# bjack205/rsLQR

Hardware: AMD Instinct MI355X
Metric: LQR solves/sec (nx=12,nu=4,N=256,batch=1024 per GPU) (higher is better)
Workload: dtype f64; 1 GPU; nx=12 nu=4 N=256 batch=1024 per GPU, fp64, factor+solve per step; parallelism=batch-sharded x1, no data-path collective, ranks_seen=1, flags=0, schedule=reduced-fused2

## Files before the change

### rslqr_amd/build.py

```python
import concurrent.futures
import os
import re
import shutil
import subprocess
import sys

PKG = os.path.dirname(os.path.abspath(__file__))
ROOT = os.path.dirname(PKG)
CSRC = os.path.join(PKG, "csrc")
INCLUDE = os.path.join(ROOT, "include")
OBJDIR = os.path.join(PKG, "build")
LIB = os.path.join(PKG, "librslqr_amd.so")
ARCH = "gfx950"

C_SOURCES = ["containers.c", "synth.c", "json.c", "batch.c", "solver.c", "linalg.c", "stages.c"]
HIP_MAIN = "ndlqr_hip.hip"
HIP_INSTANCE = "small_instance.hip"
HIP_DEPS = ["kernels_common.hpp", "kernels_leaf.hpp", "kernels_generic.hpp", "kernels_grad.hpp", "kernels_box.hpp", "kernels_box_grad.hpp", "kernels_small.hpp", "kernels_bottom_reduced.hpp", "kernels_dpp.hpp", "kernels_rowbcast.hpp", "kernels_mfma.hpp", "kernels_reduced_mfma.hpp",
            "hip_context.hpp", "launch_small.hpp", "small_instances.def"]


def small_instances():
    text = open(os.path.join(CSRC, "small_instances.def")).read()
    return [(int(a), int(b)) for a, b in re.findall(r"^NDLQR_SMALL_INSTANCE\((\d+),\s*(\d+)\)", text, flags=re.M)]


def _hipcc():
    for cand in (os.environ.get("HIPCC"), shutil.which("hipcc"), "/opt/rocm/bin/hipcc"):
        if cand and os.path.exists(cand):
            return cand
    raise RuntimeError("hipcc not found (set HIPCC)")


def _newer(target, deps):
    if not os.path.exists(target):
        return True
    t = os.path.getmtime(target)
    return any(os.path.exists(d) and os.path.getmtime(d) > t for d in deps)


def _run(cmd):
    proc = subprocess.run(cmd, stdout=subprocess.PIPE, stderr=subprocess.STDOUT, text=True)
    if proc.returncode != 0:
        sys.stderr.write(" ".join(cmd) + "\n" + proc.stdout + "\n")
        raise RuntimeError("build step failed: " + cmd[0])
    if proc.stdout.strip():
        sys.stderr.write(proc.stdout)


def build(force=False, verbose=False):
    os.makedirs(OBJDIR, exist_ok=True)
    headers = [os.path.join(INCLUDE, h) for h in ("ndlqr.h", "ndlqr_hip.h")]
    me = os.path.abspath(__file__)
    hipcc = _hipcc()
    hip_flags = [hipcc, "--offload-arch=" + ARCH, "-std=c++17", "-O3", "-ffp-contract=off", "-fPIC", "-Wall",
                 "-Wno-pass-failed",
                 "-I" + INCLUDE, "-I" + CSRC] + os.environ.get("NDLQR_EXTRA_HIPFLAGS", "").split()
    hip_deps = [me] + headers + [os.path.join(CSRC, h) for h in HIP_DEPS]
    jobs, objs = [], []
    for src in C_SOURCES:
        s = os.path.join(CSRC, src)
        o = os.path.join(OBJDIR, src + ".o")
        if force or _newer(o, [s, me] + headers):
            jobs.append(("cc " + src, ["gcc", "-std=gnu11", "-O2", "-g0", "-fPIC", "-Wall", "-Wextra",
                                       "-I" + INCLUDE, "-c", s, "-o", o]))
        objs.append(o)
    s = os.path.join(CSRC, HIP_MAIN)
    o = os.path.join(OBJDIR, HIP_MAIN + ".o")
    if force or _newer(o, [s] + hip_deps):
        jobs.append(("hipcc " + HIP_MAIN, hip_flags + ["-c", s, "-o", o]))
    objs.append(o)
    s = os.path.join(CSRC, HIP_INSTANCE)
    for nx, nu in small_instances():
        o = os.path.join(OBJDIR, "small_%d_%d.o" % (nx, nu))
        if force or _newer(o, [s] + hip_deps):
            jobs.append(("hipcc small instance (%d,%d)" % (nx, nu),
                         hip_flags + ["-DNDLQR_INST_NX=%d" % nx, "-DNDLQR_INST_NU=%d" % nu, "-c", s, "-o", o]))
        objs.append(o)
    if jobs:
        workers = max(1, min(len(jobs), (os.cpu_count() or 2)))
        with concurrent.futures.ThreadPoolExecutor(max_workers=workers) as pool:
            futures = {pool.submit(_run, cmd): label for label, cmd in jobs}
            for fut in concurrent.futures.as_completed(futures):
                fut.result()
                if verbose:
                    print(futures[fut])
    if force or _newer(LIB, objs):
        if verbose:
            print("link", os.path.basename(LIB))
        _run([hipcc, "--offload-arch=" + ARCH, "-shared", "-fPIC", "-o", LIB] + objs + ["-lm", "-lpthread"])
    return LIB


if __name__ == "__main__":
    print(build(force="--force" in sys.argv, verbose=True))
```

### rslqr_amd/csrc/kernels_bottom_reduced.hpp

```cpp
#pragma once
#include "kernels_dpp.hpp"
#include "kernels_small.hpp"

namespace ndlqr {

typedef double acc4_t __attribute__((ext_vector_type(4)));

template <int NX>
struct McPitch {
  static constexpr int SP = 18, WP = 17;
};

template <int NX, class Hook>
__device__ __forceinline__ void factor_tail_mc(const int lane, const acc4_t& c, const double (&ra)[(NX + 3) / 4],
                                               const double (&rb)[(NX + 3) / 4], const double* Wm, acc4_t& X0,
                                               acc4_t& X1, Hook hook) {
  constexpr int KS = (NX + 3) / 4, WP = McPitch<NX>::WP;
  int lane_o = lane;
  asm volatile("" : "+v"(lane_o));
  const int li = lane_o & 15, lk = lane_o >> 4;
  double wt[KS], wa[KS], b0[KS];
#pragma unroll
  for (int q = 0; q < KS; ++q) {
    wt[q] = Wm[(4 * q + lk) * WP + li];
    wa[q] = Wm[li * WP + 4 * q + lk];
    b0[q] = li == NX ? c[q] : ra[q];
  }
  const acc4_t zero = {0.0, 0.0, 0.0, 0.0};
  acc4_t Y0 = zero, Y1 = zero;
#pragma unroll
  for (int q = 0; q < KS; ++q) {
    Y0 = __builtin_amdgcn_mfma_f64_16x16x4f64(wa[q], b0[q], Y0, 0, 0, 0);
    Y1 = __builtin_amdgcn_mfma_f64_16x16x4f64(wa[q], rb[q], Y1, 0, 0, 0);
  }
  X0 = zero; X1 = zero;
  double y0[KS], y1[KS];
#pragma unroll
  for (int q = 0; q < KS; ++q) {
    y0[q] = Y0[q]; y1[q] = Y1[q];
    X0 = __builtin_amdgcn_mfma_f64_16x16x4f64(wt[q], Y0[q], X0, 0, 0, 0);
    X1 = __builtin_amdgcn_mfma_f64_16x16x4f64(wt[q], Y1[q], X1, 0, 0, 0);
  }
  hook(y0, y1, Y0, Y1);
}

template <int NX>
struct McWyLayout {
  static constexpr int SP = McPitch<NX>::SP, WP = McPitch<NX>::WP, KS = (NX + 3) / 4, YP = 17, TILE = 4 * KS * YP;
  static constexpr int Y0 = 0, Y1 = TILE, W = 2 * TILE;
  static constexpr int SIZE = 2 * TILE + 16 * WP > 16 * SP ? 2 * TILE + 16 * WP : 16 * SP;
  static_assert(2 * NX + 1 <= 32, "the panel fits the lanes of two DPP rows");
};
template <int NX>
__device__ __forceinline__ bool chol_wy_mc(const int lane_in, const acc4_t& c, double* buf, double (&w)[NX],
                                           double* lstore) {
  using P = McWyLayout<NX>;
  constexpr int SP = P::SP, YP = P::YP, KS = P::KS;
  static_assert(P::YP == P::WP, "one store stride for both kinds of lanes");
  int lane = lane_in;
  asm volatile("" : "+v"(lane));
  const int li = lane & 15, lk = lane >> 4, h = lane & 31;
  const int ri = li < NX ? li : NX - 1;
#pragma unroll
  for (int g = 0; g < 4; ++g) buf[(lk + 4 * g) * SP + li] = c[g];
  wave_lds_sync();
  double acc[NX];
  if constexpr (NX % 2 == 0) {
#pragma unroll
    for (int j = 0; j < NX; j += 2) {
      const double2 t = *reinterpret_cast<const double2*>(&buf[ri * SP + j]);
      acc[j] = t.x; acc[j + 1] = t.y;
    }
  } else {
#pragma unroll
    for (int j = 0; j < NX; ++j) acc[j] = buf[ri * SP + j];
  }
  if (lk >= 2) {
#pragma unroll
    for (int k = 0; k < NX; ++k) w[k] = (k == li) ? 1.0 : 0.0;
  } else if (h == NX) {
#pragma unroll
    for (int k = 0; k < NX; ++k) w[k] = buf[k * SP + NX];
  }
  const bool bad = rb_chol_inv<NX, false>(li, acc, w);
  wave_lds_sync();
  {
    const int ycol = h <= NX ? P::Y0 + h : P::Y1 + (h <= 2 * NX ? h - NX - 1 : YP - 1);
    double* dst = buf + (lk < 2 ? ycol : P::W + li);
#pragma unroll
    for (int k = 0; k < NX; ++k) dst[k * YP] = w[k];
    if constexpr (4 * KS > NX) {
#pragma unroll
      for (int e0 = 0; e0 < (4 * KS - NX) * YP; e0 += 32) {
        const int e = e0 + h;
        if (e < (4 * KS - NX) * YP && lk < 2) {
          buf[P::Y0 + NX * YP + e] = 0.0;
          buf[P::Y1 + NX * YP + e] = 0.0;
        }
      }
    }
#pragma unroll
    for (int e0 = 0; e0 < (16 - NX) * P::WP; e0 += 32) {
      const int e = e0 + h;
      if (e < (16 - NX) * P::WP && lk >= 2) buf[P::W + NX * P::WP + e] = 0.0;
    }
  }
  if (lstore && lane < NX) store_row<NX>(lstore + li * NX, acc);
  wave_lds_sync();
  return bad;
}

template <int NX, class Hook>
__device__ __forceinline__ void tail_wy_mc(const int lane, const double* buf, acc4_t& X0, acc4_t& X1, Hook hook) {
  using P = McWyLayout<NX>;
  constexpr int KS = P::KS;
  int lane_o = lane;
  asm volatile("" : "+v"(lane_o));
  const int li = lane_o & 15, lk = lane_o >> 4;
  double wt[KS], y0[KS], y1[KS];
  acc4_t Z0 = {0.0, 0.0, 0.0, 0.0}, Z1 = {0.0, 0.0, 0.0, 0.0};
#pragma unroll
  for (int q = 0; q < KS; ++q) {
    wt[q] = buf[P::W + (4 * q + lk) * P::WP + li];
    y0[q] = buf[P::Y0 + (4 * q + lk) * P::YP + li];
    y1[q] = buf[P::Y1 + (4 * q + lk) * P::YP + li];
    Z0[q] = y0[q]; Z1[q] = y1[q];
  }
  const acc4_t zero = {0.0, 0.0, 0.0, 0.0};
  X0 = zero; X1 = zero;
#pragma unroll
  for (int q = 0; q < KS; ++q) {
    X0 = __builtin_amdgcn_mfma_f64_16x16x4f64(wt[q], y0[q], X0, 0, 0, 0);
    X1 = __builtin_amdgcn_mfma_f64_16x16x4f64(wt[q], y1[q], X1, 0, 0, 0);
  }
  hook(y0, y1, Z0, Z1);
}

template <int NX>
struct McPairLayout {
  static constexpr int SP = McPitch<NX>::SP, WP = McPitch<NX>::WP;
  static constexpr int SCR_A = 0, SCR_B = 16 * SP, W_A = 32 * SP, W_B = 0, SIZE = 32 * SP + 16 * WP;
  static_assert(16 * WP <= 16 * SP, "W_B fits over the S-bar tile of A");
};
template <int NX>
__device__ __forceinline__ bool chol_pair_mc(const int lane_in, const acc4_t& cA, const acc4_t& cB, double* buf,
                                             double* lstoreA, double* lstoreB) {
  using P = McPairLayout<NX>;
  constexpr int SP = P::SP, WP = P::WP;
  int lane = lane_in;
  asm volatile("" : "+v"(lane));
  const int li = lane & 15, lk = lane >> 4;
  const int ri = li < NX ? li : NX - 1;
#pragma unroll
  for (int g = 0; g < 4; ++g) {
    buf[P::SCR_A + (lk + 4 * g) * SP + li] = cA[g];
    buf[P::SCR_B + (lk + 4 * g) * SP + li] = cB[g];
  }
  wave_lds_sync();
  const double* mine = buf + (lk < 2 ? P::SCR_A : P::SCR_B) + ri * SP;
  double acc[NX], w[NX];
  if constexpr (NX % 2 == 0) {
#pragma unroll
    for (int j = 0; j < NX; j += 2) {
      const double2 t = *reinterpret_cast<const double2*>(&mine[j]);
      acc[j] = t.x; acc[j + 1] = t.y;
    }
  } else {
#pragma unroll
    for (int j = 0; j < NX; ++j) acc[j] = mine[j];
  }
  const bool bad = rb_chol_inv<NX>(li, acc, w);
  wave_lds_sync();
  {
    double* wdst = buf + (lk < 2 ? P::W_A : P::W_B) + li;
#pragma unroll
    for (int r = 0; r < NX; ++r) wdst[r * WP] = w[r];
#pragma unroll
    for (int e0 = 0; e0 < (16 - NX) * WP; e0 += 32) {
      const int e = e0 + (lane & 31);
      if (e < (16 - NX) * WP) buf[(lk < 2 ? P::W_A : P::W_B) + NX * WP + e] = 0.0;
    }
  }
  if (lstoreA && lane < NX) store_row<NX>(lstoreA + li * NX, acc);
  if (lstoreB && lane >= 32 && lane < 32 + NX) store_row<NX>(lstoreB + li * NX, acc);
  wave_lds_sync();
  return bad;
}
// ... 42 lines not shown
    const int x = lk >> 1;
    double* ydst = buf + (h <= NX ? P::tile(x, 0) + h : P::tile(x, 1) + (h <= 2 * NX ? h - NX - 1 : YP - 1));
#pragma unroll
    for (int k = 0; k < NX; ++k) ydst[k * YP] = w[k];
    if constexpr (4 * KS > NX) {
#pragma unroll
      for (int e0 = 0; e0 < (4 * KS - NX) * YP; e0 += 16) {
        const int e = e0 + li;
        if (e < (4 * KS - NX) * YP) buf[P::tile(x, lk & 1) + NX * YP + e] = 0.0;
      }
    }
  }
  if ((lk & 1) == 0 && li < NX) {
    double* lr = (lk == 0 ? lrecA : lrecB) + li * (li + 1) / 2;
#pragma unroll
    for (int c = 0; c < NX; ++c)
      if (c <= li) lr[c] = acc[c];
  }
  wave_lds_sync();
  return bad;
}

template <int NX, bool N00, bool N01, bool N10, bool N11>
__device__ __forceinline__ void gram_mc(const double (&R0)[(NX + 3) / 4], const double (&R1)[(NX + 3) / 4],
                                        const acc4_t& X0, const acc4_t& X1, acc4_t& g00, acc4_t& g01, acc4_t& g10,
                                        acc4_t& g11) {
  constexpr int KS = (NX + 3) / 4;
  const acc4_t zero = {0.0, 0.0, 0.0, 0.0};
  g00 = zero; g01 = zero; g10 = zero; g11 = zero;
#pragma unroll
  for (int q = 0; q < KS; ++q) {
    if constexpr (N00) g00 = __builtin_amdgcn_mfma_f64_16x16x4f64(R0[q], X0[q], g00, 0, 0, 0);
    if constexpr (N01) g01 = __builtin_amdgcn_mfma_f64_16x16x4f64(R0[q], X1[q], g01, 0, 0, 0);
    if constexpr (N10) g10 = __builtin_amdgcn_mfma_f64_16x16x4f64(R1[q], X0[q], g10, 0, 0, 0);
    if constexpr (N11) g11 = __builtin_amdgcn_mfma_f64_16x16x4f64(R1[q], X1[q], g11, 0, 0, 0);
  }
}

template <int NX> __device__ __forceinline__ constexpr bool rows_all(int g) { return 4 * g + 3 < NX; }
template <int NX> __device__ __forceinline__ constexpr bool rows_none(int g) { return 4 * g >= NX; }

template <int NX>
__device__ __forceinline__ void store_record_mc(double* __restrict__ myrec, const int lane, const bool ha,
                                                const bool hb, const acc4_t& X0, const acc4_t& X1) {
  constexpr int NN = NX * NX;
  const int li = lane & 15, lk = lane >> 4;
  if (li < NX) {
    if (ha) {
#pragma unroll
      for (int g = 0; g < 4; ++g) {
        const int r = lk + 4 * g;
        if (!rows_none<NX>(g) && (rows_all<NX>(g) || r < NX)) myrec[r * NX + li] = X0[g];
      }
    }
    if (hb) {
#pragma unroll
      for (int g = 0; g < 4; ++g) {
        const int r = lk + 4 * g;
        if (!rows_none<NX>(g) && (rows_all<NX>(g) || r < NX)) myrec[NN + r * NX + li] = X1[g];
      }
    }
  } else if (li == NX) {
#pragma unroll
    for (int g = 0; g < 4; ++g) {
      const int r = lk + 4 * g;
      if (!rows_none<NX>(g) && (rows_all<NX>(g) || r < NX)) myrec[2 * NN + r] = X0[g];
    }
  }
}

struct StorePlain { __device__ __forceinline__ void operator()(double* p, double v) const { *p = v; } };
struct StoreThrough {
  __device__ __forceinline__ void operator()(double* p, double v) const {
    __hip_atomic_store(p, v, __ATOMIC_RELAXED, __HIP_MEMORY_SCOPE_AGENT);
  }
};
struct AddAtomic { __device__ __forceinline__ void operator()(double* p, double v) const { atomicAdd(p, v); } };

template <int NX, class Put, class Set>
__device__ __forceinline__ void push_mc(const int lane, const bool hasA, const bool hasB, const bool leftchild,
                                        const RedSlot<NX>& sa, const RedSlot<NX>& sb, const acc4_t& g00,
                                        const acc4_t& g01, const acc4_t& g11, const acc4_t& pa, const acc4_t& pb01,
                                        const acc4_t& pb11, Put put, Set set) {
  const int li = lane & 15, lk = lane >> 4;
  if (hasA && li <= NX) {
#pragma unroll
    for (int g = 0; g < 4; ++g) {
      const int r = lk + 4 * g;
      if (!rows_none<NX>(g) && (rows_all<NX>(g) || r < NX) && (li <= r || li == NX))
        put(li < NX ? sa.DR() + r * (r + 1) / 2 + li : sa.gR() + r, g00[g] + pa[g]);
    }
  }
  if (hasB && li < NX) {
#pragma unroll
    for (int g = 0; g < 4; ++g) {
      const int r = lk + 4 * g;
      if (!rows_none<NX>(g) && (rows_all<NX>(g) || r < NX) && li <= r) put(sb.DL() + r * (r + 1) / 2 + li, g11[g] + pb11[g]);
    }
    if (lk == NX % 4) put(sb.gL() + li, g01[NX / 4] + pb01[NX / 4]);
    if (hasA) {
#pragma unroll
      for (int g = 0; g < 4; ++g) {
        const int r = lk + 4 * g;
        if (!rows_none<NX>(g) && (rows_all<NX>(g) || r < NX))
          set(leftchild ? sb.CA() + li * NX + r : sa.CB() + r * NX + li, g01[g]);
      }
    }
  }
}

template <int NX, int NU, int WP, bool NEXT = true, class Init>
__device__ __forceinline__ acc4_t leaf_tile_mc(const int lane, const bool first, const double* am, const double* q0,
                                               const double* q1, const double* z0, const double* z1, Init init) {
  constexpr int W = NX + NU, KS = (W + 3) / 4;
  const int li = lane & 15, lk = lane >> 4;
  const int ri = li < NX ? li : NX - 1;
  double w1[4], za[4], zb[4], in0[4], av[KS], wk[KS], zraw[KS];
#pragma unroll
  for (int g = 0; g < 4; ++g) {
    const int i = lk + 4 * g, ic = i < NX ? i : NX - 1;
    if constexpr (NEXT) { w1[g] = q1[ic]; za[g] = z1[ic]; zb[g] = z1[NX + ic]; }
    else { w1[g] = 0.0; za[g] = 0.0; zb[g] = 0.0; }
    in0[g] = init(g);
  }
#pragma unroll
  for (int q = 0; q < KS; ++q) {
    const int kq = 4 * q + lk, k = kq < W ? kq : W - 1;
    const bool fx = first && k < NX;
    av[q] = am[ri * WP + k]; wk[q] = q0[k]; zraw[q] = z0[fx ? k : NX + k];
  }
  acc4_t c;
#pragma unroll
  for (int g = 0; g < 4; ++g) {
    const int i = lk + 4 * g;
    c[g] = (li == NX ? -fma(zb[g], w1[g], za[g]) : ((i == li) ? w1[g] : 0.0)) + in0[g];
  }
#pragma unroll
  for (int q = 0; q < KS; ++q) {
    const int kq = 4 * q + lk, k = kq < W ? kq : W - 1;
    const bool kin = kq < W, fx = first && k < NX;
    const double sv = fx ? 0.0 : av[q] * wk[q];
    const double zc = fx ? -zraw[q] : zraw[q] * wk[q];
    const double bsel = li == NX ? zc : sv;
    if constexpr (W % 4 == 0) c = __builtin_amdgcn_mfma_f64_16x16x4f64(av[q], bsel, c, 0, 0, 0);
    else c = __builtin_amdgcn_mfma_f64_16x16x4f64(kin ? av[q] : 0.0, bsel, c, 0, 0, 0);
  }
  return c;
}

template <int NX>
__device__ __forceinline__ constexpr int rb_lrec_offset() { return (NX * (NX + 1) / 2 + 1) / 2 * 2; }
template <int NX>
__device__ __forceinline__ double* rb_lrec(double* rec, const Dims& d, const int b, const int s) {
  return rec + ((size_t)b * d.N + (s - 1)) * (2 * NX * NX + NX) + rb_lrec_offset<NX>();
}
template <int NX>
__device__ __forceinline__ const double* rb_lrec(const double* rec, const Dims& d, const int b, const int s) {
  return rec + ((size_t)b * d.N + (s - 1)) * (2 * NX * NX + NX) + rb_lrec_offset<NX>();
}

template <int NX>
__device__ __forceinline__ double* lstore_of(const int store_l, double* F, double* rec, const Dims& d, const int b,
                                             const int level, const int s) {
  return store_l == 2 ? rb_lrec<NX>(rec, d, b, s) : (store_l ? Fblk(F, d, b, level, s + 1) : nullptr);
}

template <int NX, int NU, bool BOTTOM = true>
struct alignas(16) ReducedLds {
  static constexpr int W = NX + NU, ROWS = 2 * NX + NU, WP = (W % 2 == 0) ? W + 2 : W;
  static constexpr int SLOT = RedSlot<NX>::SIZE, NSC = McWyLayout<NX>::SIZE;
  static constexpr int NB0 = BOTTOM ? 4 * NX * WP : 0, NB1 = SLOT + NX * WP;
  static constexpr int NB2 = BOTTOM ? McPairLayout<NX>::SIZE : 0;
  static constexpr int NB3 = BOTTOM ? McPairYLayout<NX>::SIZE : 0;
  static constexpr int NB01 = (NB0 > NB1 ? NB0 : NB1) > NSC ? (NB0 > NB1 ? NB0 : NB1) : NSC;
  static constexpr int NB23 = NB2 > NB3 ? NB2 : NB3;
  static constexpr int NBUF = NB01 > NB23 ? NB01 : NB23;
  static constexpr int NRQ = BOTTOM ? 4 * W : (W + NX + 1) / 2 * 2, NRH = BOTTOM ? 4 * ROWS : (NX + W + 2 * NX + 1) / 2 * 2;
  double buf[NBUF];
  double rq[NRQ];
  double rh[NRH];
#ifdef NDLQR_DEV_LDS_PAD
  double dev_pad[BOTTOM ? NDLQR_DEV_LDS_PAD / 8 : 1];
#endif
};

template <int NX, int NU, bool TREE, class LdsT, bool EXT = false>
__device__ __forceinline__ void reduced_separator_mc(const Dims& d, const int l, const int base, const int b,
                                                     const int lane, const double* __restrict__ AB,
                                                     const double* __restrict__ QR,
                                                     const double* __restrict__ rhs, double* red,
                                                     double* __restrict__ rec, double* F, int* __restrict__ info,
                                                     const int store_l, LdsT& lds, const double* slot_ext = nullptr) {
  constexpr int W = NX + NU, NN = NX * NX, KSN = (NX + 3) / 4;
  constexpr int WP = ReducedLds<NX, NU>::WP, SLOT = RedSlot<NX>::SIZE;
  const double* slot = EXT ? slot_ext : lds.buf;
  double* abs_ = lds.buf + SLOT;
  double* rq = lds.rq;
  double* zs = lds.rh;
  static_assert(LdsT::NRQ >= W + NX && LdsT::NRH >= NX + W + 2 * NX, "the shared arrays are large enough for a level");
  const int N = d.N;
  const int T = 2 << l, s = base + (1 << l) - 1;
  const bool hasA = base > 0, hasB = base + T < N;
  const int li = lane & 15, lk = lane >> 4;
  const int ri = li < NX ? li : NX - 1;
  SEG_INIT();
  const bool leftchild = (base & T) == 0;
  const RedSlot<NX> sa = red_slot<NX>(red, d, b, hasA ? base - 1 : s);
  const RedSlot<NX> sb = red_slot<NX>(red, d, b, hasB ? base + T - 1 : s);

  {
    const double* sl = red_slot<NX>(red, d, b, s).p;
    const double* abm = AB + ((size_t)b * N + s) * NX * W;
    const double* qr = QR + ((size_t)b * N + s) * W;
    const double* r0 = rhs + ((size_t)b * N + s) * (2 * NX + NU);
    constexpr int NS = SLOT / 2, IS = (NS + 63) / 64, NA = NX * W, IA = (NA + 63) / 64;
    constexpr int NQ = W + NX, IQ = (NQ + 63) / 64, NR = NX + W + 2 * NX, IR = (NR + 63) / 64;
    static_assert(SLOT % 2 == 0, "slot copied as 16-byte words");
    double2 ts[IS];
    double ta[IA], tq[IQ], tr[IR];
#pragma unroll
    for (int it = 0; it < (EXT ? 0 : IS); ++it) {
      const int e = lane + 64 * it, ec = e < NS ? e : NS - 1;
      if constexpr (TREE) {
        ts[it].x = __hip_atomic_load(sl + 2 * ec, __ATOMIC_RELAXED, __HIP_MEMORY_SCOPE_AGENT);
        ts[it].y = __hip_atomic_load(sl + 2 * ec + 1, __ATOMIC_RELAXED, __HIP_MEMORY_SCOPE_AGENT);
      } else {
        ts[it] = reinterpret_cast<const double2*>(sl)[ec];
      }
    }
#pragma unroll
    for (int it = 0; it < IA; ++it) { const int e = lane + 64 * it; ta[it] = abm[e < NA ? e : NA - 1]; }
#pragma unroll
    for (int it = 0; it < IQ; ++it) { const int e = lane + 64 * it; tq[it] = qr[e < NQ ? e : NQ - 1]; }
#pragma unroll
    for (int it = 0; it < IR; ++it) { const int e = lane + 64 * it; tr[it] = r0[e < NR ? e : NR - 1]; }
#pragma unroll
    for (int it = 0; it < (EXT ? 0 : IS); ++it) {
      const int e = lane + 64 * it, ec = e < NS ? e : NS - 1;
      reinterpret_cast<double2*>(lds.buf)[ec] = ts[it];
    }
#pragma unroll
    for (int it = 0; it < IA; ++it) {
      const int e = lane + 64 * it, ec = e < NA ? e : NA - 1, row = ec / W, c = ec - row * W;
      abs_[row * WP + c] = ta[it];
    }
#pragma unroll
    for (int it = 0; it < IQ; ++it) { const int e = lane + 64 * it, ec = e < NQ ? e : NQ - 1; rq[ec] = 1.0 / tq[it]; }
#pragma unroll
    for (int it = 0; it < IR; ++it) { const int e = lane + 64 * it, ec = e < NR ? e : NR - 1; zs[ec] = tr[it]; }
  }
  wave_lds_sync();
  constexpr int TRI = RedSlot<NX>::TRI;
  const double *DL = slot, *DR = slot + TRI, *CA = slot + 2 * TRI, *CB = slot + 2 * TRI + NN;
  const double *gL = slot + 2 * TRI + 2 * NN, *gR = slot + 2 * TRI + 2 * NN + NX;

  const acc4_t c0 = leaf_tile_mc<NX, NU, WP>(lane, false, abs_, rq, rq + W, zs, zs + NX + W, [&](int g) {
    const int i = lk + 4 * g, ic = i < NX ? i : NX - 1;
    const int tix = RedSlot<NX>::tri(ic, ri);
    const double dd = DL[tix] + DR[tix], gg = gL[ic] + gR[ic];
    return -(li == NX ? gg : dd);
  });
  double wcol[NX];
  {
    const int h = lane & 31;
    const bool is_a = h < NX, is_b = h > NX && h <= 2 * NX;
    const double* src = is_a ? CA + h : CB + (is_b ? h - NX - 1 : 0);
    const double sign = ((is_a && hasA) || (is_b && hasB)) ? -1.0 : 0.0;
#pragma unroll
    for (int k = 0; k < NX; ++k) wcol[k] = src[k * NX] * sign;
  }
  wave_lds_sync();
  SEG(9);

  acc4_t X0, X1, unused;
  if (chol_wy_mc<NX>(lane, c0, lds.buf, wcol, lstore_of<NX>(store_l, F, rec, d, b, l, s)) && lane == 0)
    flag_failure(info, d, b);
  SEG(31);
  tail_wy_mc<NX>(lane, lds.buf, X0, X1,
                 [&](const double (&R0)[KSN], const double (&R1)[KSN], const acc4_t& Z0, const acc4_t& Z1) {
                   acc4_t g00, g01, g11;
                   gram_mc<NX, true, true, false, true>(R0, R1, Z0, Z1, g00, g01, unused, g11);
                   const acc4_t zero = {0.0, 0.0, 0.0, 0.0};
                   if constexpr (TREE)
                     push_mc<NX>(lane, hasA, hasB, leftchild, sa, sb, g00, g01, g11, zero, zero, zero, AddAtomic(),
                                 StoreThrough());
                   else
                     push_mc<NX>(lane, hasA, hasB, leftchild, sa, sb, g00, g01, g11, zero, zero, zero, AddAtomic(),
                                 StorePlain());
                 });
  SEG(13);
  store_record_mc<NX>(rec + ((size_t)b * N + s) * (2 * NN + NX), lane, hasA, hasB, X0, X1);
#ifdef NDLQR_SEGTIME
  __builtin_amdgcn_s_waitcnt(0);
#endif
  SEG(12);
}

template <int NX, int NU>
__global__ __launch_bounds__(64) __attribute__((amdgpu_waves_per_eu(4))) void reduced_level_mc(
    Dims d, int l, const double* __restrict__ AB, const double* __restrict__ QR, const double* __restrict__ rhs,
    double* red, double* __restrict__ rec, double* F, int* __restrict__ info, const int store_l) {
  __shared__ ReducedLds<NX, NU, false> lds;
  reduced_separator_mc<NX, NU, false>(d, l, (blockIdx.x + d.xoff) * (2 << l), blockIdx.y, threadIdx.x, AB, QR, rhs, red, rec, F,
                                      info, store_l, lds);
}


template <int NX, int NU>
__device__ __forceinline__ void reduced_eliminate_pass_mc(const Dims& d, const int base, const int b, const int lane,
                                                          const acc4_t& c_leaf, const double* slot,
                                                          int* __restrict__ info, double* buf) {
  constexpr int NN = NX * NX, TRI = RedSlot<NX>::TRI;
  const int N = d.N, T = 8;
  const bool hasA = base > 0, hasB = base + T < N;
  const int li = lane & 15, lk = lane >> 4, ri = li < NX ? li : NX - 1;
  const double *DL = slot, *DR = slot + TRI, *CA = slot + 2 * TRI, *CB = slot + 2 * TRI + NN;
  const double *gL = slot + 2 * TRI + 2 * NN, *gR = slot + 2 * TRI + 2 * NN + NX;
  acc4_t c0;
#pragma unroll
  for (int g = 0; g < 4; ++g) {
    const int i = lk + 4 * g, ic = i < NX ? i : NX - 1;
    const int tix = RedSlot<NX>::tri(ic, ri);
    const double dd = DL[tix] + DR[tix], gg = gL[ic] + gR[ic];
    c0[g] = c_leaf[g] - (li == NX ? gg : dd);
  }
  double wcol[NX];
  {
    const int h = lane & 31;
    const bool is_a = h < NX, is_b = h > NX && h <= 2 * NX;
    const double* src = is_a ? CA + h : CB + (is_b ? h - NX - 1 : 0);
    const double sign = ((is_a && hasA) || (is_b && hasB)) ? -1.0 : 0.0;
#pragma unroll
    for (int k = 0; k < NX; ++k) wcol[k] = src[k * NX] * sign;
  }
  wave_lds_sync();
  if (chol_wy_mc<NX>(lane, c0, buf, wcol, nullptr) && lane == 0) flag_failure(info, d, b);
}
template <int NX, int NU>
__device__ __forceinline__ void reduced_eliminate_tail_mc(const Dims& d, const int base, const int b, const int lane,
                                                          const bool gram, double* red, double* __restrict__ rec,
                                                          const double* buf) {
  using P = McWyLayout<NX>;
  constexpr int NN = NX * NX, KS = P::KS;
  const int N = d.N, T = 8, s = base + 3;
  const bool hasA = base > 0, hasB = base + T < N, leftchild = (base & T) == 0;
  const int li = lane & 15, lk = lane >> 4;
  double y0[KS], y1[KS];
  acc4_t Z0 = {0.0, 0.0, 0.0, 0.0}, Z1 = {0.0, 0.0, 0.0, 0.0};
#pragma unroll
  for (int q = 0; q < KS; ++q) {
    y0[q] = buf[P::Y0 + (4 * q + lk) * P::YP + li];
    y1[q] = buf[P::Y1 + (4 * q + lk) * P::YP + li];
    Z0[q] = y0[q]; Z1[q] = y1[q];
  }
  if (gram) {
    const RedSlot<NX> sa = red_slot<NX>(red, d, b, hasA ? base - 1 : s);
    const RedSlot<NX> sb = red_slot<NX>(red, d, b, hasB ? base + T - 1 : s);
    acc4_t g00, g01, g11, unused;
    gram_mc<NX, true, true, false, true>(y0, y1, Z0, Z1, g00, g01, unused, g11);
    const acc4_t zero = {0.0, 0.0, 0.0, 0.0};
    push_mc<NX>(lane, hasA, hasB, leftchild, sa, sb, g00, g01, g11, zero, zero, zero, AddAtomic(), StorePlain());
  } else {
    double wt[KS];
#pragma unroll
    for (int q = 0; q < KS; ++q) wt[q] = buf[P::W + (4 * q + lk) * P::WP + li];
    acc4_t X0 = {0.0, 0.0, 0.0, 0.0}, X1 = {0.0, 0.0, 0.0, 0.0};
#pragma unroll
    for (int q = 0; q < KS; ++q) {
      X0 = __builtin_amdgcn_mfma_f64_16x16x4f64(wt[q], y0[q], X0, 0, 0, 0);
      X1 = __builtin_amdgcn_mfma_f64_16x16x4f64(wt[q], y1[q], X1, 0, 0, 0);
    }
    store_record_mc<NX>(rec + ((size_t)b * N + s) * (2 * NN + NX), lane, hasA, hasB, X0, X1);
  }
}

template <int NX, int NU, bool TREE, bool REDIRECT>
__device__ __forceinline__ void bottom_group_mc(const Dims& d, const int k0, const int b, const int lane,
                                                const double* __restrict__ AB, const double* __restrict__ QR,
                                                const double* __restrict__ rhs, double* red, double* __restrict__ rec,
                                                double* F, int* __restrict__ info, const int store_l, const int compact0,
                                                ReducedLds<NX, NU>& lds, double* slotA, double* slotB,
                                                const bool with_m = false, acc4_t* c_m = nullptr);
template <int NX, int NU>
__global__ __launch_bounds__(128) __attribute__((amdgpu_waves_per_eu(4))) void bottom8_reduced_mc(
    Dims d, const double* __restrict__ AB, const double* __restrict__ QR, const double* __restrict__ rhs, double* red,
    double* __restrict__ rec, int* __restrict__ info) {
  __shared__ ReducedLds<NX, NU> lds[2];
  __shared__ __attribute__((aligned(16))) double mslot[RedSlot<NX>::SIZE];
  const int wave = __builtin_amdgcn_readfirstlane(threadIdx.x >> 6), b = blockIdx.y;
  const int kw = (blockIdx.x + d.xoff) * 8;
  int lane = threadIdx.x & 63;
  for (int e = threadIdx.x; e < RedSlot<NX>::SIZE; e += 128) mslot[e] = 0.0;
  __syncthreads();
  acc4_t c_m = {0.0, 0.0, 0.0, 0.0};
  bottom_group_mc<NX, NU, false, true>(d, kw + 4 * wave, b, lane, AB, QR, rhs, red, rec, nullptr, info, 0, 1, lds[wave],
                                       wave == 1 ? mslot : nullptr, wave == 0 ? mslot : nullptr, wave == 0, &c_m);
  asm volatile("s_waitcnt vmcnt(0)" ::: "memory");
  __syncthreads();
  asm volatile("" : "+v"(lane));
  if (wave == 0) reduced_eliminate_pass_mc<NX, NU>(d, kw, b, lane, c_m, mslot, info, lds[0].buf);
  __syncthreads();
  reduced_eliminate_tail_mc<NX, NU>(d, kw, b, lane, wave == 0, red, rec, lds[0].buf);
}

template <int NX>
__device__ __forceinline__ void backsub_top_body(const Dims& d, const int b, const int t,
                                                 const double* __restrict__ recs, double* __restrict__ ytop,
                                                 double* ytop_lds, const int bp = -1, const double* zsep = nullptr);
template <int NX, int NU>
__global__ __launch_bounds__(256) __attribute__((amdgpu_waves_per_eu(4))) void reduced_top_mc(Dims d, const int l0, const double* __restrict__ AB,
                                                      const double* __restrict__ QR, const double* __restrict__ rhs,
                                                      double* red, double* __restrict__ rec, double* F,
                                                      int* __restrict__ info, const int store_l,
                                                      double* __restrict__ ytop) {
  __shared__ ReducedLds<NX, NU, false> lds[4];
  const int wave = __builtin_amdgcn_readfirstlane(threadIdx.x >> 6), b = blockIdx.x;
  for (int l = l0, s0 = 0; l < d.K;) {
    int lane = threadIdx.x & 63;
    asm volatile("" : "+v"(lane));
    const int cnt = d.N >> (l + 1);
    if (wave + s0 < cnt)
      reduced_separator_mc<NX, NU, true>(d, l, (wave + s0) * (2 << l), b, lane, AB, QR, rhs, red, rec, F, info, store_l,
                                         lds[wave]);
    s0 += 4;
    if (s0 < cnt) continue;
    s0 = 0;
    ++l;
    asm volatile("s_waitcnt vmcnt(0)" ::: "memory");
    __syncthreads();
  }
  if (ytop) backsub_top_body<NX>(d, b, threadIdx.x, rec, ytop, reinterpret_cast<double*>(&lds[0]), -1, nullptr);
}

template <int NX, int NU, bool TREE, bool REDIRECT>
__device__ __forceinline__ void bottom_group_mc(const Dims& d, const int k0, const int b, const int lane,
                                                const double* __restrict__ AB, const double* __restrict__ QR,
                                                const double* __restrict__ rhs, double* red, double* __restrict__ rec,
                                                double* F, int* __restrict__ info, const int store_l, const int compact0,
                                                ReducedLds<NX, NU>& lds, double* slotA, double* slotB,
                                                const bool with_m, acc4_t* c_m) {
  constexpr int W = NX + NU, ROWS = 2 * NX + NU, NN = NX * NX, KSN = (NX + 3) / 4;
  constexpr int REC = 2 * NN + NX;
  constexpr int WP = ReducedLds<NX, NU>::WP;
  double* abs_ = lds.buf;
  double* rq = lds.rq;
  double* rh = lds.rh;
  const int N = d.N;
  const int li = lane & 15, lk = lane >> 4;
  const int ri = li < NX ? li : NX - 1;
  const bool hasA = k0 > 0, hasB = k0 + 4 < N;
  SEG_INIT();

  {
    const double* abm = AB + ((size_t)b * N + k0) * NX * W;
    const double* q0 = QR + ((size_t)b * N + k0) * W;
    const double* r0 = rhs + ((size_t)b * N + k0) * ROWS;
    constexpr int NQ = 4 * W, IQ = (NQ + 63) / 64, NR = 4 * ROWS, IR = (NR + 63) / 64;
    double qv[IQ], rv[IR];
#pragma unroll
    for (int it = 0; it < IQ; ++it) { const int e = lane + 64 * it; qv[it] = q0[e < NQ ? e : NQ - 1]; }
#pragma unroll
    for (int it = 0; it < IR; ++it) { const int e = lane + 64 * it; rv[it] = r0[e < NR ? e : NR - 1]; }
    if constexpr (W % 2 == 0) {
      constexpr int NA = 4 * NX * W / 2, IA = (NA + 63) / 64;
      double2 t[IA];
#pragma unroll
      for (int it = 0; it < IA; ++it) {
        const int e = lane + 64 * it;
        t[it] = reinterpret_cast<const double2*>(abm)[e < NA ? e : NA - 1];
      }
#pragma unroll
      for (int it = 0; it < IA; ++it) {
        const int e = lane + 64 * it, ec = e < NA ? e : NA - 1, row = ec / (W / 2), c2 = ec - row * (W / 2);
        reinterpret_cast<double2*>(&abs_[row * WP])[c2] = t[it];
      }
    } else {
      constexpr int NA = 4 * NX * W, IA = (NA + 63) / 64;
      double t[IA];
#pragma unroll
      for (int it = 0; it < IA; ++it) { const int e = lane + 64 * it; t[it] = abm[e < NA ? e : NA - 1]; }
#pragma unroll
      for (int it = 0; it < IA; ++it) { const int e = lane + 64 * it; abs_[e < NA ? e : NA - 1] = t[it]; }
    }
#pragma unroll
    for (int it = 0; it < IQ; ++it) {
      const int e = lane + 64 * it, ec = e < NQ ? e : NQ - 1, kn = ec / W, c = ec - kn * W;
      rq[ec] = 1.0 / qv[it];
      if (e < NQ && !(qv[it] > 0.0) && !(k0 + kn == N - 1 && c >= NX)) flag_failure(info, d, b);
    }
#pragma unroll
    for (int it = 0; it < IR; ++it) { const int e = lane + 64 * it; rh[e < NR ? e : NR - 1] = rv[it]; }
  }
  wave_lds_sync();
  SEG(20);

  auto none = [](int) { return 0.0; };
  acc4_t c_s0;
  if (k0 == 0) c_s0 = leaf_tile_mc<NX, NU, WP>(lane, true, abs_, rq, rq + W, rh, rh + ROWS, none);
  else c_s0 = leaf_tile_mc<NX, NU, WP>(lane, false, abs_, rq, rq + W, rh, rh + ROWS, none);
  acc4_t c_t = leaf_tile_mc<NX, NU, WP>(lane, false, abs_ + NX * WP, rq + W, rq + 2 * W, rh + ROWS, rh + 2 * ROWS, none);
  acc4_t c_s2 = leaf_tile_mc<NX, NU, WP>(lane, false, abs_ + 2 * NX * WP, rq + 2 * W, rq + 3 * W, rh + 2 * ROWS,
                                         rh + 3 * ROWS, none);
  if constexpr (REDIRECT) {
    if (with_m) {
      const double* qn = QR + ((size_t)b * N + k0 + 4) * W;
      const double* rn = rhs + ((size_t)b * N + k0 + 4) * ROWS;
      const int e = lane < 3 * NX ? lane : 3 * NX - 1;
      const double raw = e < NX ? qn[e] : rn[e - NX];
      const double val = e < NX ? 1.0 / raw : raw;
      double nw[4], nl[4], nxv[4];
#pragma unroll
      for (int g = 0; g < 4; ++g) {
        const int i = lk + 4 * g, ic = i < NX ? i : NX - 1;
        nw[g] = __shfl(val, ic, 64); nl[g] = __shfl(val, NX + ic, 64); nxv[g] = __shfl(val, 2 * NX + ic, 64);
      }
      *c_m = leaf_tile_mc<NX, NU, WP, false>(lane, false, abs_ + 3 * NX * WP, rq + 3 * W, rq, rh + 3 * ROWS, rh, none);
#pragma unroll
      for (int g = 0; g < 4; ++g) {
        const int i = lk + 4 * g;
        (*c_m)[g] += li == NX ? -fma(nxv[g], nw[g], nl[g]) : (i == li ? nw[g] : 0.0);
      }
    }
  }
  acc4_t X0, X1, unused;
  double* myrec = rec + ((size_t)b * N + k0) * REC;
  acc4_t park_a, ca_t, park_b11, cb_t;
  auto hook_s0 = [&](const double (&R0)[KSN], const double (&R1)[KSN], const acc4_t& Z0, const acc4_t& Z1) {
    acc4_t g11;
    gram_mc<NX, true, false, true, true>(R0, R1, Z0, Z1, park_a, unused, ca_t, g11);
#pragma unroll
    for (int g = 0; g < 4; ++g) c_t[g] -= (li < NX) ? g11[g] : ca_t[g];
  };
  auto hook_s2 = [&](const double (&R0)[KSN], const double (&R1)[KSN], const acc4_t& Z0, const acc4_t& Z1) {
    acc4_t g00;
    gram_mc<NX, true, true, false, true>(R0, R1, Z0, Z1, g00, cb_t, unused, park_b11);
#pragma unroll
    for (int g = 0; g < 4; ++g) c_t[g] -= g00[g];
  };

  const bool compact_path = !TREE && compact0 != 0;
  if (!TREE && compact_path) {
    double wcol[NX];
    {
      const int h = lane & 31, x = lane >> 5;
      const bool is_a = h < NX, is_b = h > NX && h <= 2 * NX;
      const int ca = is_a ? h : 0, cb = is_b ? h - NX - 1 : 0;
      const double* src = abs_ + (2 * x) * NX * WP + (is_a ? ca : NX * WP + cb * WP);
      const double* scl = rq + (2 * x) * W + (is_a ? ca : W);
      const int sstr = is_a ? WP : 1, wstr = is_a ? 0 : 1;
      const bool on = (is_a && (x == 1 || hasA)) || (is_b && (x == 0 || hasB));
      const double sign = on ? -1.0 : 0.0;
#pragma unroll
      for (int k = 0; k < NX; ++k) wcol[k] = (src[k * sstr] * scl[k * wstr]) * sign;
    }
    wave_lds_sync();
    SEG(21);
    if (chol_pair_y_mc<NX>(lane, c_s0, c_s2, lds.buf, wcol, myrec, myrec + 2 * REC) && (lane == 0 || lane == 32))
      flag_failure(info, d, b);
    SEG(30);
    using PY = McPairYLayout<NX>;
#pragma unroll
    for (int x = 0; x < 2; ++x) {
      const double* Y0 = lds.buf + PY::tile(x, 0);
      const double* Y1 = lds.buf + PY::tile(x, 1);
      double y0[KSN], y1[KSN];
      acc4_t Z0 = {0.0, 0.0, 0.0, 0.0}, Z1 = {0.0, 0.0, 0.0, 0.0};
#pragma unroll
      for (int q = 0; q < KSN; ++q) {
        y0[q] = Y0[(4 * q + lk) * PY::YP + li];
        y1[q] = Y1[(4 * q + lk) * PY::YP + li];
        Z0[q] = y0[q]; Z1[q] = y1[q];
      }
      if (x == 0) hook_s0(y0, y1, Z0, Z1); else hook_s2(y0, y1, Z0, Z1);
    }
    SEG(35);
  } else {
  double ra0[KSN], rb0[KSN], ra2[KSN], rb2[KSN];
#pragma unroll
  for (int q = 0; q < KSN; ++q) {
    const int kq = 4 * q + lk, i = kq < NX ? kq : NX - 1;
    const double a0 = abs_[i * WP + ri], b0 = abs_[(NX + ri) * WP + i];
    const double a2 = abs_[(2 * NX + i) * WP + ri], b2 = abs_[(3 * NX + ri) * WP + i];
    const double s0 = rq[ri], s1 = rq[W + i], s2 = rq[2 * W + ri], s3 = rq[3 * W + i];
    ra0[q] = hasA ? -a0 * s0 : 0.0;
    rb0[q] = -b0 * s1;
    ra2[q] = -a2 * s2;
    rb2[q] = hasB ? -b2 * s3 : 0.0;
  }
  wave_lds_sync();
  SEG(21);

  using Pair = McPairLayout<NX>;
  if (chol_pair_mc<NX>(lane, c_s0, c_s2, lds.buf, store_l ? Fblk(F, d, b, 0, k0 + 1) : nullptr,
                       store_l ? Fblk(F, d, b, 0, k0 + 3) : nullptr) &&
      (lane == 0 || lane == 32))
    flag_failure(info, d, b);
  SEG(30);
  factor_tail_mc<NX>(lane, c_s0, ra0, rb0, lds.buf + Pair::W_A, X0, X1, hook_s0);
  store_record_mc<NX>(myrec, lane, hasA, true, X0, X1);
  factor_tail_mc<NX>(lane, c_s2, ra2, rb2, lds.buf + Pair::W_B, X0, X1, hook_s2);
  store_record_mc<NX>(myrec + 2 * REC, lane, true, hasB, X0, X1);
  SEG(35);
  }
  double wcol[NX];
  {
    constexpr int TP = 17;
    static_assert(2 * 16 * TP <= ReducedLds<NX, NU>::NBUF, "both coupling tiles fit the buffer");
    double* ta = lds.buf;
    double* tb = lds.buf + 16 * TP;
    wave_lds_sync();
#pragma unroll
    for (int g = 0; g < 4; ++g) {
      ta[(lk + 4 * g) * TP + li] = -ca_t[g];
      tb[(lk + 4 * g) * TP + li] = -cb_t[g];
    }
    wave_lds_sync();
    const int h = lane & 31;
    const bool is_a = h < NX, is_b = h > NX && h <= 2 * NX;
    const double* src = is_a ? ta + h : tb + (is_b ? h - NX - 1 : 0);
#pragma unroll
    for (int k = 0; k < NX; ++k) wcol[k] = src[k * TP];
    wave_lds_sync();
  }
  const bool leftchild = (k0 & 4) == 0;
  RedSlot<NX> sa = red_slot<NX>(red, d, b, hasA ? k0 - 1 : 3);
  RedSlot<NX> sb = red_slot<NX>(red, d, b, hasB ? k0 + 3 : 3);
  if constexpr (REDIRECT) {
    if (slotA) sa.p = slotA;
    if (slotB) sb.p = slotB;
  }
  if (chol_wy_mc<NX>(lane, c_t, lds.buf, wcol, lstore_of<NX>(store_l, F, rec, d, b, 1, k0 + 1)) && lane == 0)
    flag_failure(info, d, b);
  tail_wy_mc<NX>(lane, lds.buf, X0, X1,
                 [&](const double (&R0)[KSN], const double (&R1)[KSN], const acc4_t& Z0, const acc4_t& Z1) {
                   acc4_t g00, g01, g11;
                   gram_mc<NX, true, true, false, true>(R0, R1, Z0, Z1, g00, g01, unused, g11);
// ... 54 lines not shown
```

### rslqr_amd/csrc/kernels_small.hpp

```cpp
#pragma once
#include "kernels_common.hpp"

namespace ndlqr {



template <int NX>
__device__ __forceinline__ void load_row(const double* __restrict__ p, double (&v)[NX]) {
  if constexpr (NX % 2 == 0) {
    const double2* p2 = reinterpret_cast<const double2*>(p);
#pragma unroll
    for (int k = 0; k < NX / 2; ++k) { const double2 t = p2[k]; v[2 * k] = t.x; v[2 * k + 1] = t.y; }
  } else {
#pragma unroll
    for (int k = 0; k < NX; ++k) v[k] = p[k];
  }
}
template <int NX>
__device__ __forceinline__ void store_row(double* __restrict__ p, const double (&v)[NX]) {
  if constexpr (NX % 2 == 0) {
    double2* p2 = reinterpret_cast<double2*>(p);
#pragma unroll
    for (int k = 0; k < NX / 2; ++k) p2[k] = make_double2(v[2 * k], v[2 * k + 1]);
  } else {
// ... 214 lines not shown
      }
#pragma unroll
      for (int it = 0; it < I2; ++it) {
        const int e = lane + 64 * it, ec = e < N2 ? e : N2 - 1;
        reinterpret_cast<double2*>(in.E1x)[ec] = t2[it];
        reinterpret_cast<double2*>(in.B1x)[ec] = t3[it];
      }
    } else {
      constexpr int N1 = W * NX, I1 = (N1 + 63) / 64, N2 = NN, I2 = (N2 + 63) / 64;
      double t0[I1], t1[I1], t2[I2], t3[I2];
#pragma unroll
      for (int it = 0; it < I1; ++it) {
        const int e = lane + 64 * it, ec = e < N1 ? e : N1 - 1;
        t0[it] = Es[ec]; t1[it] = Fas[ec];
      }
#pragma unroll
      for (int it = 0; it < I2; ++it) {
        const int e = lane + 64 * it, ec = e < N2 ? e : N2 - 1;
        t2[it] = E1[ec]; t3[it] = B1[ec];
      }
#pragma unroll
      for (int it = 0; it < I1; ++it) {
        const int e = lane + 64 * it, ec = e < N1 ? e : N1 - 1;
        in.Exu[ec] = t0[it]; in.Axu[ec] = t1[it];
      }
#pragma unroll
      for (int it = 0; it < I2; ++it) {
        const int e = lane + 64 * it, ec = e < N2 ? e : N2 - 1;
        in.E1x[ec] = t2[it]; in.B1x[ec] = t3[it];
      }
    }
    in.zxu[lane < W ? lane : W - 1] = zx;
    in.z1[lane < 2 * NX ? lane : 2 * NX - 1] = zl;
  }
  wave_lds_sync();
  SEG(0);
  double Lrow[NX];
  const bool bad = separator_core<NX, NU, STRICT, KEEP>(lane, ab, in, out, Lrow,
                                                       AB + ((size_t)b * N + s) * NX * W, W,
                                                       (!LAMBDA_OUT && store_l) ? Fblk(F, d, b, l, s + 1) : nullptr);
  if (bad && lane == 0) flag_failure(info, d, b);
  SEG(6);

  double* myrec = rec + ((size_t)b * N + s) * (2 * NN + NX);
  const int grp = lane / NX;
  if (grp < 2) {
    const int colidx = grp == 0 ? a : bb;
    if (colidx >= 0) {
      double row[NX];
#pragma unroll
      for (int c = 0; c < NX; ++c) row[c] = out.X[gi * LD + grp * NX + c];
      store_row<NX>(myrec + grp * NN + gi * NX, row);
      if constexpr (LAMBDA_OUT) store_row<NX>(Fblk(F, d, b, colidx, s + 1) + gi * NX, row);
    }
  } else if (grp == 2) {
    const double v = out.X[gi * LD + 2 * NX];
    myrec[2 * NN + gi] = v;
    z[((size_t)b * N + s + 1) * ROWS + gi] = v;
  }
  if constexpr (LAMBDA_OUT) { if (lane < NX) store_row<NX>(Fblk(F, d, b, l, s + 1) + gi * NX, Lrow); }
  SEG(4);
}

template <int NX, int NU>
__device__ __forceinline__ double leaf_rhs_entry(const Dims& d, const int b, const int i, const int rr,
                                                 const double* __restrict__ QR, const double* __restrict__ rhs) {
  constexpr int W = NX + NU, ROWS = 2 * NX + NU;
  const double* r0 = rhs + ((size_t)b * d.N + i) * ROWS;
  const double* qr = QR + ((size_t)b * d.N + i) * W;
  const bool lam = rr < NX, last = (i == d.N - 1);
  if (i == 0) {
    if (lam) return fma(-qr[rr], r0[rr], -r0[NX + rr]);
    if (rr < 2 * NX) return -r0[rr - NX];
    return r0[rr] / qr[rr - NX];
  }
  if (lam) return r0[rr];
  if (rr < 2 * NX || !last) return r0[rr] / qr[rr - NX];
  return r0[rr];
}

template <int NX>
struct RedSlot {
  static constexpr int NN = NX * NX, TRI = NX * (NX + 1) / 2, USED = 2 * TRI + 2 * NN + 2 * NX, SIZE = (USED + 15) / 16 * 16;
  double* p;
  __device__ __forceinline__ double* DL() const { return p; }
  __device__ __forceinline__ double* DR() const { return p + TRI; }
  __device__ __forceinline__ double* CA() const { return p + 2 * TRI; }
  __device__ __forceinline__ double* CB() const { return p + 2 * TRI + NN; }
  __device__ __forceinline__ double* gL() const { return p + 2 * TRI + 2 * NN; }
  __device__ __forceinline__ double* gR() const { return p + 2 * TRI + 2 * NN + NX; }
  __host__ __device__ static constexpr int tri(const int r, const int c) { return r >= c ? r * (r + 1) / 2 + c : c * (c + 1) / 2 + r; }
};
template <int NX>
__device__ __forceinline__ RedSlot<NX> red_slot(double* red, const Dims& d, const int b, const int t) {
  return RedSlot<NX>{red + ((size_t)b * (d.N >> 2) + (t >> 2)) * RedSlot<NX>::SIZE};
}

template <int NX, int LDF, bool STRICT>
__device__ __forceinline__ void row_update(double (&E)[NX], double (&Ca)[NX], double (&Cb)[NX], double& zz,
                                           const double* fa, const double* fb, const double* zsp,
                                           const int zstride, const bool has_a, const bool has_b,
                                           const bool left, const bool active) {
  (void)left;
#pragma unroll
  for (int c = 0; c < NX; ++c) E[c] = active ? E[c] : 0.0;
  if (has_a) {
#pragma unroll
    for (int k = 0; k < NX; ++k)
#pragma unroll
      for (int c = 0; c < NX; ++c) Ca[c] = mad<STRICT>(-E[k], fa[k * LDF + c], Ca[c]);
  }
  if (has_b) {
#pragma unroll
    for (int k = 0; k < NX; ++k)
#pragma unroll
      for (int c = 0; c < NX; ++c) Cb[c] = mad<STRICT>(-E[k], fb[k * LDF + c], Cb[c]);
  }
#pragma unroll
  for (int k = 0; k < NX; ++k) zz = mad<STRICT>(-E[k], zsp[k * zstride], zz);
}

template <int NX, int LDF, bool STRICT>
__device__ __forceinline__ void row_update_live(double (&E)[NX], double (&C)[NX], double& zz,
                                                const double* f_live, const double* f_new, const double* zsp,
                                                const bool has_live, const bool has_new, const bool active,
                                                const bool take_sep, const int r, const bool e_is_created) {
  double D[NX];
#pragma unroll
  for (int c = 0; c < NX; ++c) { E[c] = active ? E[c] : 0.0; D[c] = 0.0; }
  if (has_live) {
#pragma unroll
    for (int k = 0; k < NX; ++k)
#pragma unroll
      for (int c = 0; c < NX; ++c) C[c] = mad<STRICT>(-E[k], f_live[k * LDF + c], C[c]);
  }
  if (has_new) {
#pragma unroll
    for (int k = 0; k < NX; ++k)
#pragma unroll
      for (int c = 0; c < NX; ++c) D[c] = mad<STRICT>(-E[k], f_new[k * LDF + c], D[c]);
  }
#pragma unroll
  for (int k = 0; k < NX; ++k) zz = mad<STRICT>(-E[k], zsp[k * LDF], zz);
  if (take_sep) {
#pragma unroll
    for (int c = 0; c < NX; ++c) {
      if (has_live) C[c] = f_live[r * LDF + c];
      if (has_new) D[c] = f_new[r * LDF + c];
    }
    zz = zsp[r * LDF];
  }
#pragma unroll
  for (int c = 0; c < NX; ++c) {
    const double cn = C[c], dn = D[c];
    E[c] = e_is_created ? dn : cn;
    C[c] = e_is_created ? cn : dn;
  }
}

template <int NX>
__device__ __forceinline__ void rotate_roles(double (&E)[NX], double (&Ca)[NX], double (&Cb)[NX],
                                             const bool left_child) {
  if (left_child) {
#pragma unroll
    for (int c = 0; c < NX; ++c) { E[c] = Cb[c]; Cb[c] = 0.0; }
  } else {
#pragma unroll
    for (int c = 0; c < NX; ++c) { E[c] = Ca[c]; Ca[c] = 0.0; }
  }
}

template <int NX, int NU>
struct SchurShape {
// ... 732 lines not shown
```

Before: 1.806 million solves/s.

## Trim address arithmetic, sign multiplies and redundant zeroing in reduced bottom kernels

Several small micro-optimizations land in the reduced bottom-level kernels. The reduction-slot push now uses precomputed unsigned offsets with incremental strides instead of per-element triangular index math. A fast path skips the sign multiply when both children are present. The LDS loader updates row and column incrementally instead of dividing. The per-block slot zeroing and its barrier now run only for boundary blocks. These target ALU and sync overhead, but the conditional zeroing assumes interior blocks never read stale slot data.

```diff
diff --git a/rslqr_amd/build.py b/rslqr_amd/build.py
--- a/rslqr_amd/build.py
+++ b/rslqr_amd/build.py
@@ -48,14 +48,18 @@
         sys.stderr.write(proc.stdout)
 
 
+def hip_flags():
+    return [_hipcc(), "--offload-arch=" + ARCH, "-std=c++17", "-O3", "-ffp-contract=off", "-fPIC", "-Wall",
+            "-Wno-pass-failed",
+            "-I" + INCLUDE, "-I" + CSRC] + os.environ.get("NDLQR_EXTRA_HIPFLAGS", "").split()
+
+
 def build(force=False, verbose=False):
     os.makedirs(OBJDIR, exist_ok=True)
     headers = [os.path.join(INCLUDE, h) for h in ("ndlqr.h", "ndlqr_hip.h")]
     me = os.path.abspath(__file__)
     hipcc = _hipcc()
-    hip_flags = [hipcc, "--offload-arch=" + ARCH, "-std=c++17", "-O3", "-ffp-contract=off", "-fPIC", "-Wall",
-                 "-Wno-pass-failed",
-                 "-I" + INCLUDE, "-I" + CSRC] + os.environ.get("NDLQR_EXTRA_HIPFLAGS", "").split()
+    flags = hip_flags()
     hip_deps = [me] + headers + [os.path.join(CSRC, h) for h in HIP_DEPS]
     jobs, objs = [], []
     for src in C_SOURCES:
@@ -68,14 +72,14 @@
     s = os.path.join(CSRC, HIP_MAIN)
     o = os.path.join(OBJDIR, HIP_MAIN + ".o")
     if force or _newer(o, [s] + hip_deps):
-        jobs.append(("hipcc " + HIP_MAIN, hip_flags + ["-c", s, "-o", o]))
+        jobs.append(("hipcc " + HIP_MAIN, flags + ["-c", s, "-o", o]))
     objs.append(o)
     s = os.path.join(CSRC, HIP_INSTANCE)
     for nx, nu in small_instances():
         o = os.path.join(OBJDIR, "small_%d_%d.o" % (nx, nu))
         if force or _newer(o, [s] + hip_deps):
             jobs.append(("hipcc small instance (%d,%d)" % (nx, nu),
-                         hip_flags + ["-DNDLQR_INST_NX=%d" % nx, "-DNDLQR_INST_NU=%d" % nu, "-c", s, "-o", o]))
+                         flags + ["-DNDLQR_INST_NX=%d" % nx, "-DNDLQR_INST_NU=%d" % nu, "-c", s, "-o", o]))
         objs.append(o)
     if jobs:
         workers = max(1, min(len(jobs), (os.cpu_count() or 2)))
diff --git a/rslqr_amd/csrc/kernels_bottom_reduced.hpp b/rslqr_amd/csrc/kernels_bottom_reduced.hpp
--- a/rslqr_amd/csrc/kernels_bottom_reduced.hpp
+++ b/rslqr_amd/csrc/kernels_bottom_reduced.hpp
@@ -97,12 +97,8 @@
           buf[P::Y0 + NX * YP + e] = 0.0;
           buf[P::Y1 + NX * YP + e] = 0.0;
         }
-      }
-    }
-#pragma unroll
-    for (int e0 = 0; e0 < (16 - NX) * P::WP; e0 += 32) {
-      const int e = e0 + h;
-      if (e < (16 - NX) * P::WP && lk >= 2) buf[P::W + NX * P::WP + e] = 0.0;
+        if (e < (4 * KS - NX) * P::WP && lk >= 2) buf[P::W + NX * P::WP + e] = 0.0;
+      }
     }
   }
   if (lstore && lane < NX) store_row<NX>(lstore + li * NX, acc);
@@ -311,28 +307,33 @@
                                         const RedSlot<NX>& sa, const RedSlot<NX>& sb, const acc4_t& g00,
                                         const acc4_t& g01, const acc4_t& g11, const acc4_t& pa, const acc4_t& pb01,
                                         const acc4_t& pb11, Put put, Set set) {
-  const int li = lane & 15, lk = lane >> 4;
+  using S = RedSlot<NX>;
+  const unsigned li = lane & 15, lk = lane >> 4;
+  const unsigned tri0 = lk * (lk + 1) / 2 + li;
   if (hasA && li <= NX) {
+    const unsigned o0 = li < NX ? S::OFF_DR + tri0 : S::OFF_GR + lk, step = li < NX ? lk : 1;
 #pragma unroll
     for (int g = 0; g < 4; ++g) {
-      const int r = lk + 4 * g;
+      const unsigned r = lk + 4 * g;
       if (!rows_none<NX>(g) && (rows_all<NX>(g) || r < NX) && (li <= r || li == NX))
-        put(li < NX ? sa.DR() + r * (r + 1) / 2 + li : sa.gR() + r, g00[g] + pa[g]);
+        put(sa.p + (o0 + 4 * g * step + (li < NX ? 8 * g * g + 2 * g : 0)), g00[g] + pa[g]);
     }
   }
   if (hasB && li < NX) {
 #pragma unroll
     for (int g = 0; g < 4; ++g) {
-      const int r = lk + 4 * g;
-      if (!rows_none<NX>(g) && (rows_all<NX>(g) || r < NX) && li <= r) put(sb.DL() + r * (r + 1) / 2 + li, g11[g] + pb11[g]);
+      const unsigned r = lk + 4 * g;
+      if (!rows_none<NX>(g) && (rows_all<NX>(g) || r < NX) && li <= r)
+        put(sb.p + (S::OFF_DL + tri0 + 4 * g * lk + (8 * g * g + 2 * g)), g11[g] + pb11[g]);
     }
     if (lk == NX % 4) put(sb.gL() + li, g01[NX / 4] + pb01[NX / 4]);
     if (hasA) {
+      double* cpl = leftchild ? sb.p : sa.p;
+      const unsigned c0 = leftchild ? S::OFF_CA + li * NX + lk : S::OFF_CB + lk * NX + li, cstep = leftchild ? 4 : 4 * NX;
 #pragma unroll
       for (int g = 0; g < 4; ++g) {
-        const int r = lk + 4 * g;
-        if (!rows_none<NX>(g) && (rows_all<NX>(g) || r < NX))
-          set(leftchild ? sb.CA() + li * NX + r : sa.CB() + r * NX + li, g01[g]);
+        const unsigned r = lk + 4 * g;
+        if (!rows_none<NX>(g) && (rows_all<NX>(g) || r < NX)) set(cpl + (c0 + g * cstep), g01[g]);
       }
     }
   }
@@ -494,9 +495,14 @@
     const int h = lane & 31;
     const bool is_a = h < NX, is_b = h > NX && h <= 2 * NX;
     const double* src = is_a ? CA + h : CB + (is_b ? h - NX - 1 : 0);
-    const double sign = ((is_a && hasA) || (is_b && hasB)) ? -1.0 : 0.0;
-#pragma unroll
-    for (int k = 0; k < NX; ++k) wcol[k] = src[k * NX] * sign;
+    if (hasA && hasB) {
+#pragma unroll
+      for (int k = 0; k < NX; ++k) wcol[k] = -src[k * NX];
+    } else {
+      const double sign = ((is_a && hasA) || (is_b && hasB)) ? -1.0 : 0.0;
+#pragma unroll
+      for (int k = 0; k < NX; ++k) wcol[k] = src[k * NX] * sign;
+    }
   }
   wave_lds_sync();
   SEG(9);
@@ -558,9 +564,14 @@
     const int h = lane & 31;
     const bool is_a = h < NX, is_b = h > NX && h <= 2 * NX;
     const double* src = is_a ? CA + h : CB + (is_b ? h - NX - 1 : 0);
-    const double sign = ((is_a && hasA) || (is_b && hasB)) ? -1.0 : 0.0;
-#pragma unroll
-    for (int k = 0; k < NX; ++k) wcol[k] = src[k * NX] * sign;
+    if (hasA && hasB) {
+#pragma unroll
+      for (int k = 0; k < NX; ++k) wcol[k] = -src[k * NX];
+    } else {
+      const double sign = ((is_a && hasA) || (is_b && hasB)) ? -1.0 : 0.0;
+#pragma unroll
+      for (int k = 0; k < NX; ++k) wcol[k] = src[k * NX] * sign;
+    }
   }
   wave_lds_sync();
   if (chol_wy_mc<NX>(lane, c0, buf, wcol, nullptr) && lane == 0) flag_failure(info, d, b);
@@ -619,8 +630,10 @@
   const int wave = __builtin_amdgcn_readfirstlane(threadIdx.x >> 6), b = blockIdx.y;
   const int kw = (blockIdx.x + d.xoff) * 8;
   int lane = threadIdx.x & 63;
-  for (int e = threadIdx.x; e < RedSlot<NX>::SIZE; e += 128) mslot[e] = 0.0;
-  __syncthreads();
+  if (kw == 0 || kw + 8 >= d.N) {
+    for (int e = threadIdx.x; e < RedSlot<NX>::SIZE; e += 128) mslot[e] = 0.0;
+    __syncthreads();
+  }
   acc4_t c_m = {0.0, 0.0, 0.0, 0.0};
   bottom_group_mc<NX, NU, false, true>(d, kw + 4 * wave, b, lane, AB, QR, rhs, red, rec, nullptr, info, 0, 1, lds[wave],
                                        wave == 1 ? mslot : nullptr, wave == 0 ? mslot : nullptr, wave == 0, &c_m);
@@ -698,10 +711,16 @@
         const int e = lane + 64 * it;
         t[it] = reinterpret_cast<const double2*>(abm)[e < NA ? e : NA - 1];
       }
+      constexpr int H = W / 2, DR = 64 / H, DC = 64 % H;
+      int row = lane / H, c2 = lane - row * H;
 #pragma unroll
       for (int it = 0; it < IA; ++it) {
-        const int e = lane + 64 * it, ec = e < NA ? e : NA - 1, row = ec / (W / 2), c2 = ec - row * (W / 2);
-        reinterpret_cast<double2*>(&abs_[row * WP])[c2] = t[it];
+        double2* dst = reinterpret_cast<double2*>(&abs_[row * WP]) + c2;
+        if (64 * it + 63 >= NA)
+          dst = lane + 64 * it < NA ? dst : reinterpret_cast<double2*>(&abs_[(4 * NX - 1) * WP]) + (H - 1);
+        *dst = t[it];
+        row += DR; c2 += DC;
+        if (DC != 0 && c2 >= H) { c2 -= H; ++row; }
       }
     } else {
       constexpr int NA = 4 * NX * W, IA = (NA + 63) / 64;
@@ -777,10 +796,15 @@
       const double* src = abs_ + (2 * x) * NX * WP + (is_a ? ca : NX * WP + cb * WP);
       const double* scl = rq + (2 * x) * W + (is_a ? ca : W);
       const int sstr = is_a ? WP : 1, wstr = is_a ? 0 : 1;
-      const bool on = (is_a && (x == 1 || hasA)) || (is_b && (x == 0 || hasB));
-      const double sign = on ? -1.0 : 0.0;
-#pragma unroll
-      for (int k = 0; k < NX; ++k) wcol[k] = (src[k * sstr] * scl[k * wstr]) * sign;
+      if (hasA && hasB) {
+#pragma unroll
+        for (int k = 0; k < NX; ++k) wcol[k] = -(src[k * sstr] * scl[k * wstr]);
+      } else {
+        const bool on = (is_a && (x == 1 || hasA)) || (is_b && (x == 0 || hasB));
+        const double sign = on ? -1.0 : 0.0;
+#pragma unroll
+        for (int k = 0; k < NX; ++k) wcol[k] = (src[k * sstr] * scl[k * wstr]) * sign;
+      }
     }
     wave_lds_sync();
     SEG(21);
diff --git a/rslqr_amd/csrc/kernels_small.hpp b/rslqr_amd/csrc/kernels_small.hpp
--- a/rslqr_amd/csrc/kernels_small.hpp
+++ b/rslqr_amd/csrc/kernels_small.hpp
@@ -320,13 +320,15 @@
 template <int NX>
 struct RedSlot {
   static constexpr int NN = NX * NX, TRI = NX * (NX + 1) / 2, USED = 2 * TRI + 2 * NN + 2 * NX, SIZE = (USED + 15) / 16 * 16;
+  static constexpr int OFF_DL = 0, OFF_DR = TRI, OFF_CA = 2 * TRI, OFF_CB = 2 * TRI + NN, OFF_GL = 2 * TRI + 2 * NN,
+                       OFF_GR = 2 * TRI + 2 * NN + NX;
   double* p;
-  __device__ __forceinline__ double* DL() const { return p; }
-  __device__ __forceinline__ double* DR() const { return p + TRI; }
-  __device__ __forceinline__ double* CA() const { return p + 2 * TRI; }
-  __device__ __forceinline__ double* CB() const { return p + 2 * TRI + NN; }
-  __device__ __forceinline__ double* gL() const { return p + 2 * TRI + 2 * NN; }
-  __device__ __forceinline__ double* gR() const { return p + 2 * TRI + 2 * NN + NX; }
+  __device__ __forceinline__ double* DL() const { return p + OFF_DL; }
+  __device__ __forceinline__ double* DR() const { return p + OFF_DR; }
+  __device__ __forceinline__ double* CA() const { return p + OFF_CA; }
+  __device__ __forceinline__ double* CB() const { return p + OFF_CB; }
+  __device__ __forceinline__ double* gL() const { return p + OFF_GL; }
+  __device__ __forceinline__ double* gR() const { return p + OFF_GR; }
   __host__ __device__ static constexpr int tri(const int r, const int c) { return r >= c ? r * (r + 1) / 2 + c : c * (c + 1) / 2 + r; }
 };
 template <int NX>
```

Measured after the change: 1.838 million solves/s (median of 6 runs). 1.02x the previous value.
